# QZ1-boy/FCVSR

Measured on AMD Instinct MI355X. Metric: SR frames/sec (7-frame window, 4x 180x320->720x1280) + PSNR vs ref, higher is better.
Workload: dtype bf16

## Files before the change

fcvsr_amd/csrc/fft.hip:

```cpp
#include <stdlib.h>
#include <mutex>
#include "common.h"

namespace fcvsr {

struct FftPlan {
  int N;
  int nfac;
  int fac[20];
  unsigned magic[20];
};

static bool make_plan(int N, FftPlan* p) {
  p->N = N;
  p->nfac = 0;
  int n = N;
  while (n % 8 == 0) { p->fac[p->nfac++] = 8; n /= 8; }
  while (n % 4 == 0) { p->fac[p->nfac++] = 4; n /= 4; }
  while (n % 2 == 0) { p->fac[p->nfac++] = 2; n /= 2; }
  while (n % 9 == 0) { p->fac[p->nfac++] = 9; n /= 9; }
  for (int f = 3; f <= n; f += 2) {
    while (n % f == 0) {
      if (p->nfac >= 20) return false;
      p->fac[p->nfac++] = f;
// ... 153 lines not shown
  int cur = 0;
  int Ns = 1;
  for (int s = 0; s < plan.nfac; ++s) {
    const int r = plan.fac[s];
    const float* xr = lds + cur * 2 * NL;
    const float* xi = xr + NL;
    float* yr = lds + (cur ^ 1) * 2 * NL;
    float* yi = yr + NL;
    const unsigned mg = plan.magic[s];
    if (r == 8) stage_radix<8, INV>(xr, xi, yr, yi, tw, N, Ns, mg, L, logL);
    else if (r == 9) stage_radix<9, INV>(xr, xi, yr, yi, tw, N, Ns, mg, L, logL);
    else if (r == 4) stage_radix<4, INV>(xr, xi, yr, yi, tw, N, Ns, mg, L, logL);
    else if (r == 2) stage_radix<2, INV>(xr, xi, yr, yi, tw, N, Ns, mg, L, logL);
    else if (r == 3) stage_radix<3, INV>(xr, xi, yr, yi, tw, N, Ns, mg, L, logL);
    else if (r == 5) stage_radix<5, INV>(xr, xi, yr, yi, tw, N, Ns, mg, L, logL);
    else if (r > 1) stage_generic(xr, xi, yr, yi, tw, N, Ns, r, L, logL);
    if (r > 1) {
      __syncthreads();
      cur ^= 1;
    }
    Ns *= r;
  }
  return cur;
}

__device__ __forceinline__ void xcd_line_chunk(int* line, int* chunk) {
  const int nchunk = gridDim.x;
  const int lin = blockIdx.y * nchunk + blockIdx.x;
  const int grp = lin / (8 * nchunk), rem = lin - grp * (8 * nchunk);
  *line = grp * 8 + (rem & 7);
  *chunk = rem >> 3;
}

__device__ __forceinline__ float ld_act(const float* base, long long idx, int dt) {
  if (dt == FCVSR_F32) return base[idx];
  const unsigned short u = reinterpret_cast<const unsigned short*>(base)[idx];
  if (dt == FCVSR_BF16) return __uint_as_float((unsigned)u << 16);
  return (float)__builtin_bit_cast(_Float16, u);
}

__device__ __forceinline__ float4 ld_act4(const float* base, long long idx, int dt) {
  if (dt == FCVSR_F32) return *reinterpret_cast<const float4*>(base + idx);
  const uint2 v = *reinterpret_cast<const uint2*>(reinterpret_cast<const unsigned short*>(base) + idx);
  if (dt == FCVSR_BF16)
    return make_float4(__uint_as_float(v.x << 16), __uint_as_float(v.x & 0xffff0000u), __uint_as_float(v.y << 16),
                       __uint_as_float(v.y & 0xffff0000u));
  typedef __attribute__((ext_vector_type(2))) _Float16 h2;
  const h2 a = __builtin_bit_cast(h2, v.x), b = __builtin_bit_cast(h2, v.y);
  return make_float4((float)a[0], (float)a[1], (float)b[0], (float)b[1]);
}

__global__ __launch_bounds__(512) void rfft_rows_kernel(View src, int src_dt, int n, int H, int W, int L, float* spec,
                                                        long long ps, int im_off, int re_off, FftPlan plan, int vec, int nbatch) {
  extern __shared__ __align__(16) float lds[];
  const int NL = W * L;
  int row, chunk;
  xcd_line_chunk(&row, &chunk);
  const int b = row / H, y = row % H;
  if (b >= nbatch) return;
  const int c0 = chunk * 2 * L;
  const int Wf = W / 2 + 1;
  make_twiddles(lds + 4 * NL, W, false);
  const long long sp = (long long)b * src.sb + (long long)y * src.sy;
  const int logL = 31 - __clz(L);
  if (vec) {
    const int G4 = L >> 1;
// ... 372 lines not shown
      const float* mk = masks + (long long)m * N * Wf + kx;
      float mv[R1];
#pragma unroll
      for (int q = 0; q < R1; ++q) mv[q] = mk[(j + q * R2) * Wf];
      Cx v[R1];
#pragma unroll
      for (int q = 0; q < R1; ++q) v[q] = live ? Cx{raw[q].r * mv[q], raw[q].i * mv[q]} : Cx{0.f, 0.f};
      Dft<R1, true>::run(v);
#pragma unroll
      for (int p = 0; p < R1; ++p) {
        const int idx = (j * R1 + p) * L + l;
        zr[idx] = v[p].r;
        zi[idx] = v[p].i;
      }
    }
    __syncthreads();
    if (j < R1) {
      Cx v[R2];
      stage2_load<R1, R2, true>(zr, zi, tw, j, l, L, v);
      if (live) {
        float* ob = out + (long long)m * out_band_stride + col0;
#pragma unroll
        for (int p = 0; p < R2; ++p) {
          float* px = ob + (long long)(j + p * R1) * rstride;
          px[re_off] = v[p].r;
          px[im_off] = v[p].i;
        }
      }
    }
    __syncthreads();
  }
}

template <int DT>
__device__ __forceinline__ Cx ld_pair(const float* base, long long idx) {
  if (DT == FCVSR_F32) { const float2 v = *reinterpret_cast<const float2*>(base + idx); return Cx{v.x, v.y}; }
  const unsigned v = *reinterpret_cast<const unsigned*>(reinterpret_cast<const unsigned short*>(base) + idx);
  if (DT == FCVSR_BF16) return Cx{__uint_as_float(v << 16), __uint_as_float(v & 0xffff0000u)};
  typedef __attribute__((ext_vector_type(2))) _Float16 h2;
  const h2 h = __builtin_bit_cast(h2, v);
  return Cx{(float)h[0], (float)h[1]};
}

template <int R1, int R2, int SDT>
__global__ __launch_bounds__(512, 4) void rfft_rows2_kernel(View src, int n, int H, int logL, float* spec, long long ps,
                                                         int im_off, int re_off, const float2* twtab, int nbatch) {
  constexpr int N = R1 * R2, Wf = N / 2 + 1;
  extern __shared__ __align__(16) float lds[];
  const int L = 1 << logL;
  float* zr = lds;
  float* zi = lds + N * L;
  float2* tw = reinterpret_cast<float2*>(lds + 2 * N * L);
  int grp, chunk;
  xcd_line_chunk(&grp, &chunk);
  const int row0 = grp, nrows = nbatch * H;
  if (row0 >= nrows) return;
  load_twiddles(tw, twtab, N);
  const int l = threadIdx.x & (L - 1), j = threadIdx.x >> logL;
  const int ca = chunk * 2 * L + 2 * l;
  const bool live = ca < n && j < R2;
  const int lane_off = live ? j * (int)src.sx + 2 * l : 0;
  auto issue = [&](const int row, Cx* v) {
    const int b = row / H, y = row - b * H;
    const long long sp = (long long)b * src.sb + (long long)y * src.sy + chunk * 2 * L;
#pragma unroll
    for (int q = 0; q < R1; ++q) {
// ... 160 lines not shown
  return L;
}
static int ilog2(int v) { int r = 0; while ((1 << r) < v) ++r; return r; }

#define FCVSR_FFT2_DISPATCH(ts, CALL)                                                                        \
  do {                                                                                                       \
    switch ((ts).N) {                                                                                        \
      case 64: CALL(8, 8); break;     case 72: CALL(8, 9); break;     case 80: CALL(8, 10); break;           \
      case 96: CALL(8, 12); break;    case 128: CALL(8, 16); break;   case 144: CALL(12, 12); break;         \
      case 160: CALL(10, 16); break;  case 180: CALL(12, 15); break;  case 192: CALL(12, 16); break;         \
      case 240: CALL(15, 16); break;  case 256: CALL(16, 16); break;  case 320: CALL(16, 20); break;         \
    }                                                                                                        \
  } while (0)
#define FCVSR_FFT2_DISPATCH_COLS(ts, CALL)                                                                   \
  do {                                                                                                       \
    switch ((ts).N) {                                                                                        \
      case 64: CALL(8, 8); break;     case 72: CALL(8, 9); break;     case 80: CALL(8, 10); break;           \
      case 96: CALL(8, 12); break;    case 128: CALL(8, 16); break;   case 144: CALL(12, 12); break;         \
      case 160: CALL(10, 16); break;  case 180: CALL(12, 15); break;  case 192: CALL(12, 16); break;         \
      case 256: CALL(16, 16); break;                                                                         \
    }                                                                                                        \
  } while (0)
#define FCVSR_FFT2_DISPATCH_BANDS(ts, CALL)                                                                  \
  do {                                                                                                       \
    switch ((ts).N) {                                                                                        \
      case 64: CALL(8, 8); break;     case 72: CALL(8, 9); break;     case 80: CALL(8, 10); break;           \
      case 96: CALL(8, 12); break;    case 128: CALL(8, 16); break;   case 144: CALL(12, 12); break;         \
      case 160: CALL(10, 16); break;  case 180: CALL(12, 15); break;                                         \
    }                                                                                                        \
  } while (0)
static const TwoStage* two_stage_cols(int N) { return (N == 240 || N == 320) ? nullptr : two_stage(N); }
static const TwoStage* two_stage_bands(int N) { return (N == 192 || N == 240 || N == 256 || N == 320) ? nullptr : two_stage(N); }

static int launch_cols2(const TwoStage& ts, const float* in, float* out, long long ps, int im_off, int re_off, int n, int Wf,
                        int B, bool inverse, const float* mask, hipStream_t st) {
  const float2* tw = twiddle_table(ts.N, st);
  if (!tw) return FCVSR_E_ARG;
  const int L = pick_lanes2(ts, n), logL = ilog2(L);
  const int rmax = ts.R1 > ts.R2 ? ts.R1 : ts.R2;
  const dim3 grid(cdiv(n, L), (B * Wf + 7) / 8 * 8), block((rmax * L + 63) / 64 * 64);
  const size_t lds = 8ull * ts.N * L + 8ull * ts.N;
#define FCVSR_COLS2(A_, B_)                                                                                                 \
  if (inverse && mask) hipLaunchKernelGGL((fft_cols2_kernel<A_, B_, true, true>), grid, block, lds, st, in, out, ps, im_off, \
                                          re_off, n, Wf, logL, mask, tw, B);                                                 \
  else if (inverse) hipLaunchKernelGGL((fft_cols2_kernel<A_, B_, true, false>), grid, block, lds, st, in, out, ps, im_off,   \
                                       re_off, n, Wf, logL, mask, tw, B);                                                    \
  else hipLaunchKernelGGL((fft_cols2_kernel<A_, B_, false, false>), grid, block, lds, st, in, out, ps, im_off, re_off, n,   \
                          Wf, logL, mask, tw, B)
  FCVSR_FFT2_DISPATCH_COLS(ts, FCVSR_COLS2);
#undef FCVSR_COLS2
  return 0;
}

static int launch_cols2_bands(const TwoStage& ts, const float* in, float* out, long long out_band_stride, long long ps, int im_off,
                             int re_off, int n, int Wf, int B, const float* masks, int nm, hipStream_t st) {
  const float2* tw = twiddle_table(ts.N, st);
  if (!tw) return FCVSR_E_ARG;
  const int L = pick_lanes2(ts, n), logL = ilog2(L);
  const int rmax = ts.R1 > ts.R2 ? ts.R1 : ts.R2;
  const dim3 grid(cdiv(n, L), (B * Wf + 7) / 8 * 8), block((rmax * L + 63) / 64 * 64);
  const size_t lds = 8ull * ts.N * L + 8ull * ts.N;
#define FCVSR_COLS2B(A_, B_) \
  hipLaunchKernelGGL((fft_cols2_bands_kernel<A_, B_>), grid, block, lds, st, in, out, out_band_stride, ps, im_off, re_off, n, Wf, logL, masks, nm, tw, B)
  FCVSR_FFT2_DISPATCH_BANDS(ts, FCVSR_COLS2B);
#undef FCVSR_COLS2B
  return 0;
}

static int launch_rfft_rows2(const TwoStage& ts, const fcvsr_view* src, int n, int B, int H, float* spec, long long ps, int im_off,
                             int re_off, hipStream_t st) {
  const float2* tw = twiddle_table(ts.N, st);
  if (!tw) return FCVSR_E_ARG;
  const int L = pick_lanes2(ts, n / 2), logL = ilog2(L);
  const int rmax = ts.R1 > ts.R2 ? ts.R1 : ts.R2;
  const dim3 grid(cdiv(n, 2 * L), (B * H + 7) / 8 * 8), block((rmax * L + 63) / 64 * 64);
  const size_t lds = 8ull * ts.N * L + 8ull * ts.N;
#define FCVSR_ROWS2(A_, B_)                                                                                                      \
  if (src->dtype == FCVSR_F32)                                                                                                   \
    hipLaunchKernelGGL((rfft_rows2_kernel<A_, B_, FCVSR_F32>), grid, block, lds, st, to_view(*src), n, H, logL, spec, ps, im_off, \
                       re_off, tw, B);                                                                                           \
  else if (src->dtype == FCVSR_BF16)                                                                                             \
    hipLaunchKernelGGL((rfft_rows2_kernel<A_, B_, FCVSR_BF16>), grid, block, lds, st, to_view(*src), n, H, logL, spec, ps,       \
                       im_off, re_off, tw, B);                                                                                   \
  else                                                                                                                           \
    hipLaunchKernelGGL((rfft_rows2_kernel<A_, B_, FCVSR_F16>), grid, block, lds, st, to_view(*src), n, H, logL, spec, ps, im_off, \
                       re_off, tw, B)
  FCVSR_FFT2_DISPATCH(ts, FCVSR_ROWS2);
#undef FCVSR_ROWS2
  return 0;
}

static int launch_irfft_rows2(const TwoStage& ts, const float* spec, long long ps, int im_off, int re_off, int n, int B, int H,
                              const fcvsr_view* dst, float scale, hipStream_t st) {
  const float2* tw = twiddle_table(ts.N, st);
  if (!tw) return FCVSR_E_ARG;
  const int L = pick_lanes2(ts, n / 2), logL = ilog2(L);
  const int rmax = ts.R1 > ts.R2 ? ts.R1 : ts.R2;
  const dim3 grid(cdiv(n, 2 * L), (B * H + 7) / 8 * 8), block((rmax * L + 63) / 64 * 64);
  const size_t lds = 8ull * ts.N * L + 8ull * ts.N;
#define FCVSR_IROWS2(A_, B_) \
  hipLaunchKernelGGL((irfft_rows2_kernel<A_, B_>), grid, block, lds, st, spec, ps, im_off, re_off, n, H, logL, to_view(*dst), scale, tw, B)
  FCVSR_FFT2_DISPATCH(ts, FCVSR_IROWS2);
#undef FCVSR_IROWS2
  return 0;
}

static bool pair_ok(const fcvsr_view* v) {
  const int al = v->dtype == FCVSR_F32 ? 8 : 4;
  return v->sc == 1 && v->sx % 2 == 0 && v->sy % 2 == 0 && v->sb % 2 == 0 && ((uintptr_t)v->ptr % al) == 0;
}

constexpr long long kFftLdsBudget = 64 * 1024;

static int pick_lanes(int N, int n_lanes_needed) {
  int L = 32;
  while (L > 1 && (16ll * N * L + 8ll * N) > kFftLdsBudget) L >>= 1;
  while (L > 1 && L / 2 >= n_lanes_needed) L >>= 1;
  return L;
}

template <class K>
static hipError_t allow_lds(K kernel, size_t bytes) {
  return hipFuncSetAttribute((const void*)kernel, hipFuncAttributeMaxDynamicSharedMemorySize, (int)bytes);
}

}

using namespace fcvsr;

extern "C" int fcvsr_rfft2(const fcvsr_view* src, int B, int H, int W, int n, float* spec, int64_t pix_stride,
                           int im_off, int re_off, void* stream) {
  FCVSR_CHECK_ARG(src && src->ptr && spec, "null pointer");
  FCVSR_CHECK_ARG(src->dtype == FCVSR_F32 || src->dtype == FCVSR_BF16 || src->dtype == FCVSR_F16, "bad src dtype");
  FCVSR_CHECK_ARG(B > 0 && H > 0 && W > 1 && n > 0 && n <= src->c, "bad sizes");
  FftPlan pw, ph;
  FCVSR_CHECK_ARG(make_plan(W, &pw) && make_plan(H, &ph), "length has too many factors");
  const int Wf = W / 2 + 1;
  hipStream_t st = (hipStream_t)stream;
  const bool spec_ok = pix_stride % 4 == 0 && im_off % 4 == 0 && re_off % 4 == 0 && ((uintptr_t)spec % 16) == 0;
  const bool spec_pair = pix_stride % 2 == 0 && im_off % 2 == 0 && re_off % 2 == 0 && ((uintptr_t)spec % 8) == 0;
  const TwoStage* tsw = two_stage(W);
  const TwoStage* tsh = two_stage_cols(H);
  if (tsw && n % 2 == 0 && pair_ok(src) && spec_pair) {
    const int rc = launch_rfft_rows2(*tsw, src, n, B, H, spec, (long long)pix_stride, im_off, re_off, st);
    if (rc) return rc;
    FCVSR_LAUNCH_CHECK();
  } else {
    const int L = pick_lanes(W, (n + 1) / 2);
    FCVSR_CHECK_ARG(16ll * W * L + 8ll * W <= 160 * 1024, "row too long for LDS");
    const size_t lds = 16ull * W * L + 8ull * W;
    (void)allow_lds(rfft_rows_kernel, lds);
    dim3 grid(cdiv(n, 2 * L), (B * H + 7) / 8 * 8);
    const int sal = src->dtype == FCVSR_F32 ? 16 : 8;
    const int vec = (L >= 4 && n % (2 * L) == 0 && src->sc == 1 && src->sx % 4 == 0 && src->sy % 4 == 0 && src->sb % 4 == 0 &&
                     ((uintptr_t)src->ptr % sal) == 0 && spec_ok) ? 1 : 0;
    hipLaunchKernelGGL(rfft_rows_kernel, grid, dim3(512), lds, st, to_view(*src), (int)src->dtype, n, H, W, L, spec,
                       (long long)pix_stride, im_off, re_off, pw, vec, B);
    FCVSR_LAUNCH_CHECK();
  }
  if (tsh) {
    const int rc = launch_cols2(*tsh, spec, spec, (long long)pix_stride, im_off, re_off, n, Wf, B, false, nullptr, st);
    if (rc) return rc;
    FCVSR_LAUNCH_CHECK();
  } else {
    const int L = pick_lanes(H, n);
    FCVSR_CHECK_ARG(16ll * H * L + 8ll * H <= 160 * 1024, "column too long for LDS");
    const size_t lds = 16ull * H * L + 8ull * H;
    (void)allow_lds(fft_cols_kernel, lds);
    dim3 grid(cdiv(n, L), (B * Wf + 7) / 8 * 8);
    const int vec = (L >= 4 && n % L == 0 && spec_ok) ? 1 : 0;
    hipLaunchKernelGGL(fft_cols_kernel, grid, dim3(512), lds, st, (const float*)spec, spec, (long long)pix_stride, im_off,
                       re_off, n, H, Wf, L, 0, (const float*)nullptr, ph, vec, B);
    FCVSR_LAUNCH_CHECK();
  }
  return 0;
}

static int irfft_rows(const float* mid, long long pix_stride, int im_off, int re_off, int n, int B, int H, int W, const FftPlan& pw,
                      bool mid_vec, const fcvsr_view* dst, hipStream_t st) {
  const TwoStage* tsw = two_stage(W);
  const bool mid_pair = pix_stride % 2 == 0 && im_off % 2 == 0 && re_off % 2 == 0 && ((uintptr_t)mid % 8) == 0;
  if (tsw && n % 2 == 0 && pair_ok(dst) && mid_pair) {
    const int rc = launch_irfft_rows2(*tsw, mid, pix_stride, im_off, re_off, n, B, H, dst, 1.0f / ((float)H * (float)W), st);
    if (rc) return rc;
    FCVSR_LAUNCH_CHECK();
  } else {
    const int L = pick_lanes(W, (n + 1) / 2);
    FCVSR_CHECK_ARG(16ll * W * L + 8ll * W <= 160 * 1024, "row too long for LDS");
    const size_t lds = 16ull * W * L + 8ull * W;
    (void)allow_lds(irfft_rows_kernel, lds);
    dim3 grid(cdiv(n, 2 * L), (B * H + 7) / 8 * 8);
// ... 38 lines not shown

extern "C" int fcvsr_irfft2_bands(const float* spec, int64_t pix_stride, int im_off, int re_off, int B, int H, int W, int n,
                                  const float* masks, int n_bands, float* work, const fcvsr_view* dst, void* stream) {
  FCVSR_CHECK_ARG(spec && masks && work && dst && n_bands >= 1 && n_bands <= 16, "null argument / 1..16 bands");
  FCVSR_CHECK_ARG(B > 0 && H > 0 && W > 1 && n > 0, "bad sizes");
  const int Wf = W / 2 + 1;
  const long long band = (long long)B * H * Wf * pix_stride;
  hipStream_t st = (hipStream_t)stream;
  const TwoStage* tsh = two_stage_bands(H);
  if (!tsh) {
    for (int m = 0; m < n_bands; ++m) {
      const int rc = fcvsr_irfft2(spec, pix_stride, im_off, re_off, B, H, W, n, masks + (long long)m * H * Wf, work, &dst[m], stream);
      if (rc) return rc;
    }
    return 0;
  }
  for (int m = 0; m < n_bands; ++m)
    FCVSR_CHECK_ARG(dst[m].ptr && dst[m].dtype == FCVSR_F32 && n <= dst[m].c, "dst: f32 views with >= n channels");
  {
    const int rc = launch_cols2_bands(*tsh, spec, work, band, (long long)pix_stride, im_off, re_off, n, Wf, B, masks, n_bands, st);
    if (rc) return rc;
    FCVSR_LAUNCH_CHECK();
  }
  FftPlan pw;
  FCVSR_CHECK_ARG(make_plan(W, &pw), "length has too many factors");
  for (int m = 0; m < n_bands; ++m) {
    const float* mid = work + (long long)m * band;
    const bool mid_vec = pix_stride % 4 == 0 && im_off % 4 == 0 && re_off % 4 == 0 && ((uintptr_t)mid % 16) == 0;
    const int rc = irfft_rows(mid, (long long)pix_stride, im_off, re_off, n, B, H, W, pw, mid_vec, &dst[m], st);
    if (rc) return rc;
  }
  return 0;
}
```

fcvsr_amd/engine.py:

```python
from __future__ import annotations

import ctypes as C
import math
import weakref
from collections import OrderedDict
from typing import Dict, List, Optional, Tuple

import numpy as np
import torch

from . import hip
from .hip import ACT_LEAKY, ACT_NONE, ACT_PRELU, ACT_RELU, check, lib, ptr, stream_ptr, view


_MASKS: Dict[Tuple[int, int, int], torch.Tensor] = {}


def band_masks_half(Q: int, H: int, W: int) -> torch.Tensor:
    key = (Q, H, W)
    if key not in _MASKS:
        n = 1024
        step = math.sqrt((n / 2) ** 2 + (n / 2) ** 2) / Q
        d2 = (np.arange(-(n // 2), n - n // 2, 1) ** 2).astype(np.float64)
        r2 = np.power(np.sqrt(d2[:, None] + d2[None, :]), 2)
# ... 369 lines not shown
                    else:
                        s_v, v_v = view(s), view(vbuf)
                        check(L.fcvsr_warp(C.byref(cur_v), C.byref(o_v), B, H, W, C.byref(s_v), st), "fcvsr_warp")
                        check(L.fcvsr_sac_v(C.byref(s_v), C.byref(k_v), B, H, W, C.byref(v_v), st), "fcvsr_sac_v")
                        check(L.fcvsr_sac_h(C.byref(v_v), C.byref(k_v), C.byref(fv), 0.1, B, H, W, C.byref(d_v), st),
                              "fcvsr_sac_h")
                    cur = dst
        out = self._new(dev, B, H, W, n, dtype=fdt_act)
        self._conv("MGAA.conv3", [al], out, res=[x2])
        if self.taps is not None:
            self._tap(f"mgaa{tag}.off_f", off4[:B])
            self._tap(f"mgaa{tag}.off_b", off4[B:])
            self._tap(f"mgaa{tag}.sim", sim)
            o = offsets.permute(0, 3, 1, 2).reshape(B, 2, A, 2, H, W)
            self.taps[f"mgaa{tag}.offsets_f"] = o[:, 0].contiguous().clone()
            self.taps[f"mgaa{tag}.offsets_b"] = o[:, 1].contiguous().clone()
            self._tap(f"mgaa{tag}.al_f", al[..., :n])
            self._tap(f"mgaa{tag}.al_b", al[..., n:])
            self._tap(f"mgaa{tag}.out", out)
        return out

    def _mffr(self, x, out_dtype=torch.float32):
        m = self._model()
        n, Q = m.n_feats, m.Freq_Inv
        dev = x.device
        B, H, W, _ = x.shape
        Wf = W // 2 + 1
        L = lib()
        st = stream_ptr()
        par = self._par
        masks = self._mask(Q, H, W, dev)
        spec = self._new(dev, B, H, Wf, 2 * n)
        xv = view(x)
        check(L.fcvsr_rfft2(C.byref(xv), B, H, W, n, spec.data_ptr(), 2 * n, 0, n, st), "fcvsr_rfft2")
        bands = self._new(dev, Q, B, H, W, n)
        work = self._new(dev, Q, B, H, Wf, 2 * n)
        bvs = (hip.View * Q)(*[view(bands[q]) for q in range(Q)])
        check(L.fcvsr_irfft2_bands(spec.data_ptr(), 2 * n, 0, n, B, H, W, n, masks.data_ptr(), Q, work.data_ptr(), bvs, st),
              "fcvsr_irfft2_bands")
        freq = [bands[Q - 1 - i] for i in range(Q)]
        s_o = self._new(dev, B, H, W, n)
        nblk = (H * W + 255) // 256
        scratch = self._new(dev, 2 * B * nblk * n)
        sums = self._new(dev, 2, B, n)
        inv_hw = 1.0 / (H * W)
        mean_sum = self._channel_sum(freq[0])
        ab = [(par[f"MFFRblock.DivEnh_block.{i}.a"], par[f"MFFRblock.DivEnh_block.{i}.b"]) for i in range(Q)]
        staged = n % 4 == 0 and 256 % (n // 4) == 0 and all(f.data_ptr() % 16 == 0 for f in freq)
        s_f = self._new(dev, B, H, W, n) if (Q > 4 or not staged) else None
        check(L.fcvsr_divenh(0, 1, freq[0].data_ptr(), (s_f if s_f is not None else s_o).data_ptr(), s_o.data_ptr(),
                             ab[0][0].data_ptr(), ab[0][1].data_ptr(), mean_sum.data_ptr(), inv_hw, None, None, sums.data_ptr(),
                             scratch.data_ptr(), scratch.numel(), B, H, W, n, st), "fcvsr_divenh(reduce)")
        gates = []
        j0 = 0
        for i in range(Q):
            pre = f"MFFRblock.DivEnh_block.{i}"
            a, b = ab[i]
            first = 1 if i == 0 else 0
            g1 = self._ca_gate(sums[0], inv_hw, pre + ".ca", B, n)
            g2 = self._ca_gate(sums[1], inv_hw, pre + ".ca", B, n) if i > 0 else None
            gates.append((g1, g2))
            sums = self._new(dev, 2, B, n)
            nxt = i + 1 < Q
            if staged:
                sa = hip.DivEnhStageArgs()
                if j0 > 0:
                    sa.ck_s_f, sa.ck_s_o = s_f.data_ptr(), s_o.data_ptr()
                for k, j in enumerate(range(j0, i + 1)):
                    sa.f[k], sa.a[k], sa.b[k] = freq[j].data_ptr(), ab[j][0].data_ptr(), ab[j][1].data_ptr()
                    sa.g1[k], sa.g2[k] = gates[j][0].data_ptr(), ptr(gates[j][1])
                sa.mean_f_sum = mean_sum.data_ptr()
                if nxt:
# ... 381 lines not shown
```

fcvsr_amd/hip.py:

```python
from __future__ import annotations

import ctypes as C
import os
from typing import Optional, Sequence

import torch

_HERE = os.path.dirname(os.path.abspath(__file__))
LIB_PATH = os.path.join(_HERE, "lib", "libfcvsr_hip.so")

F32, BF16, F16, U8 = 0, 1, 2, 3
ACT_NONE, ACT_RELU, ACT_LEAKY, ACT_PRELU = 0, 1, 2, 3
_DT = {torch.float32: F32, torch.bfloat16: BF16, torch.float16: F16, torch.uint8: U8}


class View(C.Structure):
    _fields_ = [("ptr", C.c_void_p), ("sb", C.c_int64), ("sy", C.c_int64), ("sx", C.c_int64), ("sc", C.c_int64),
                ("c", C.c_int32), ("dtype", C.c_int32)]


class GcFinishLevel(C.Structure):
    _fields_ = [("partial", C.c_void_p), ("add", C.c_void_p), ("nparts", C.c_int32)]


# ... 2 lines not shown


class GcApplyLevel(C.Structure):
    _fields_ = [("r", C.c_void_p), ("add", C.c_void_p), ("z", C.c_void_p), ("out", C.c_void_p), ("pool", C.c_void_p),
                ("B", C.c_int32), ("H", C.c_int32), ("W", C.c_int32)]


class XscaleLevel(C.Structure):
    _fields_ = [("x", C.c_void_p), ("r", C.c_void_p), ("dn", C.c_void_p), ("up", C.c_void_p), ("out", C.c_void_p),
                ("r_scale", C.c_float), ("dn_pooled", C.c_int32), ("B", C.c_int32), ("H", C.c_int32), ("W", C.c_int32)]


class RcbTailArgs(C.Structure):
    _fields_ = [("x", C.c_void_p * 3), ("r", C.c_void_p * 3), ("z", C.c_void_p * 3), ("add", C.c_void_p * 3),
                ("out", C.c_void_p * 3), ("r1", C.c_void_p), ("u1", C.c_void_p), ("u2", C.c_void_p), ("w_up", C.c_void_p),
                ("b_up", C.c_void_p), ("w_dn", C.c_void_p), ("b_dn", C.c_void_p), ("B", C.c_int32), ("H", C.c_int32),
                ("W", C.c_int32)]


class DivEnhStageArgs(C.Structure):
    _fields_ = [("ck_s_f", C.c_void_p), ("ck_s_o", C.c_void_p), ("f", C.c_void_p * 4), ("a", C.c_void_p * 4),
                ("b", C.c_void_p * 4), ("g1", C.c_void_p * 4), ("g2", C.c_void_p * 4), ("mean_f_sum", C.c_void_p),
                ("f_next", C.c_void_p), ("a_next", C.c_void_p), ("b_next", C.c_void_p), ("out_s_f", C.c_void_p),
                ("out_s_o", C.c_void_p), ("sums", C.c_void_p), ("scratch", C.c_void_p), ("scratch_elems", C.c_int64),
                ("inv_hw", C.c_float), ("n_bands", C.c_int32), ("B", C.c_int32), ("H", C.c_int32), ("W", C.c_int32),
                ("C", C.c_int32)]


class CropDesc(C.Structure):
    _fields_ = [("src", C.c_void_p), ("pitch", C.c_int32), ("top", C.c_int32), ("left", C.c_int32), ("flags", C.c_int32)]


CROP_HFLIP, CROP_VFLIP, CROP_TRANSPOSE = 1, 2, 4


class ConvDesc(C.Structure):
    _fields_ = [("n_src", C.c_int32), ("src", View * 3), ("B", C.c_int32), ("H", C.c_int32), ("W", C.c_int32),
                ("kh", C.c_int32), ("kw", C.c_int32), ("stride", C.c_int32), ("pad", C.c_int32),
                ("cout", C.c_int32), ("weight", C.c_void_p), ("cout_pad", C.c_int32), ("bias", C.c_void_p),
                ("act", C.c_int32), ("slope", C.c_float), ("slope_ptr", C.c_void_p), ("n_res", C.c_int32),
                ("res", View * 2), ("res_scale", C.c_float * 2), ("dst", View), ("pixel_shuffle", C.c_int32),
                ("gc_wmask", C.c_void_p), ("gc_partial", C.c_void_p)]


PROFILE = None
COMPUTE_DTYPE = "f32"
DOMINANT_KERNEL = "conv_direct_kernel"


class HipError(RuntimeError):
    pass


_lib: Optional[C.CDLL] = None

_VP, _I, _I64, _F = C.c_void_p, C.c_int, C.c_int64, C.c_float
_PV = C.POINTER(View)
SIGNATURES = {
    "fcvsr_last_error": [],
    "fcvsr_last_conv_kernel": [],
    "fcvsr_conv2d_wgrad_scratch_elems": [C.c_int] * 7,
    "fcvsr_conv2d_wgrad": [C.c_void_p, C.c_void_p, C.c_int, C.c_int, C.c_int, C.c_int, C.c_int, C.c_int, C.c_int, C.c_void_p, C.c_void_p,
                           C.c_longlong, C.c_int, C.c_void_p],
    "fcvsr_conv2d_wgrad_mfma_eligible": [C.c_int] * 6,
    "fcvsr_conv2d_wgrad_mfma_scratch_elems": [C.c_int] * 7,
    "fcvsr_conv2d_wgrad_mfma": [C.c_void_p, C.c_void_p, C.c_int, C.c_int, C.c_int, C.c_int, C.c_int, C.c_int, C.c_int, C.c_void_p, C.c_void_p,
                                C.c_void_p, C.c_longlong, C.c_int, C.c_int, C.c_void_p],
    "fcvsr_abi_version": [],
    "fcvsr_device_count": [],
    "fcvsr_conv2d": [C.POINTER(ConvDesc), _VP],
    "fcvsr_conv2d_f32mfma": [C.POINTER(ConvDesc), _VP],
    "fcvsr_conv2d_f32mfma_eligible": [C.POINTER(ConvDesc)],
    "fcvsr_conv2d_mfma": [C.POINTER(ConvDesc), _I, _I, _VP],
    "fcvsr_conv2d_mfma_plan": [C.POINTER(ConvDesc), _I, _I, _I, _I, C.c_char_p, _I],
    "fcvsr_rfft2": [_PV, _I, _I, _I, _I, _VP, _I64, _I, _I, _VP],
    "fcvsr_irfft2": [_VP, _I64, _I, _I, _I, _I, _I, _I, _VP, _VP, _PV, _VP],
    "fcvsr_irfft2_bands": [_VP, _I64, _I, _I, _I, _I, _I, _I, _VP, _I, _VP, _PV, _VP],
    "fcvsr_corr_lookup": [_VP, _VP, _I64, _I, _I, _I, _I, _I, _I, _PV, _VP],
    "fcvsr_channel_sum": [_PV, _I, _I, _I, _VP, _VP, _I64, _VP],
    "fcvsr_ca_gate": [_VP, _F, _VP, _VP, _I, _I, _I, _VP, _VP],
    "fcvsr_convblk_tail": [_VP, _VP, _VP, _I, _I, _I, _I, _VP, _I64, _I, _I, _I, _I, _VP],
    "fcvsr_convblk": [_VP, _VP, _VP, _VP, _I, _VP, _VP, _VP, _I, _I, _I, _I, _VP, _VP, _I64, _VP, _I64, _I, _I, _I, _I, _VP],
    "fcvsr_warp": [_PV, _PV, _I, _I, _I, _PV, _VP],
    "fcvsr_sac_v": [_PV, _PV, _I, _I, _I, _PV, _VP],
    "fcvsr_sac_h": [_PV, _PV, _PV, _F, _I, _I, _I, _PV, _VP],
    "fcvsr_iac_step": [_PV, _PV, _PV, _PV, _F, _I, _I, _I, _PV, _VP],
    "fcvsr_feat_extract": [_PV, _I, _I, _I, _VP, _VP, _I, _VP, _VP, _VP, _I, _VP],
    "fcvsr_freq_head": [_VP, _I, _I64, _I64, _VP, _VP, _VP, _VP, _VP],
    "fcvsr_freq_mlp3": [_VP, _VP, _I, _I64, _I64, _VP, _VP, _VP, _VP, _I64, _VP],
    "fcvsr_iac_step2": [_PV, _PV, _PV, _PV, _F, _I, _I, _I, _PV, _VP],
    "fcvsr_iac_step2_fused": [_PV, _PV, _PV, _VP, _VP, _PV, _F, _I, _I, _I, _PV, _VP],
    "fcvsr_divenh": [_I, _I, _VP, _VP, _VP, _VP, _VP, _VP, _F, _VP, _VP, _VP, _VP, _I64, _I, _I, _I, _I, _VP],
    "fcvsr_divenh_apply_next": [_I, _VP, _VP, _VP, _VP, _VP, _VP, _F, _VP, _VP, _VP, _VP, _VP, _VP, _VP, _I64, _I, _I, _I, _I, _VP],
    "fcvsr_divenh_stage": [C.POINTER(DivEnhStageArgs), _VP],
    "fcvsr_scale_add": [_VP, _VP, _VP, _I, _VP, _I, _I, _I, _I, _I, _VP],
    "fcvsr_gc_context": [_VP, _VP, _VP, _VP, _I, _I, _I, _I, _VP, _VP, _I64, _VP],
    "fcvsr_gc_finish": [_VP, _I, _VP, _VP, _I, _I, _VP, _VP],
    "fcvsr_gc_apply": [_VP, _VP, _VP, _VP, _I, _F, _I, _I, _I, _I, _VP],
    "fcvsr_xscale": [_VP, _VP, _F, _VP, _VP, _VP, _I, _I, _I, _I, _I, _VP],
    "fcvsr_gc_finish_levels": [C.POINTER(GcFinishLevel), _I, _VP, _VP, _I, _I, _VP],
    "fcvsr_gc_partial_levels": [C.POINTER(GcPartialLevel), _I, _I, _VP, _I, _VP],
    "fcvsr_gc_apply_levels": [C.POINTER(GcApplyLevel), _I, _I, _I, _F, _I, _VP],
    "fcvsr_xscale_levels": [C.POINTER(XscaleLevel), _I, _I, _I, _VP],
    "fcvsr_rcb_level0": [_VP, _VP, _VP, _VP, _VP, _VP, _VP, _F, _F, _I, _I, _I, _I, _I, _VP],
    "fcvsr_rcb_tail": [C.POINTER(RcbTailArgs), _F, _I, _I, _VP],
    "fcvsr_pixel_shuffle": [_VP, _VP, _I, _I, _I, _I, _VP],
    "fcvsr_pixel_shuffle16": [_VP, _PV, _I, _I, _I, _I, _VP],
    "fcvsr_bilinear_up4": [_PV, _I, _I, _I, _PV, _VP],
    "fcvsr_tail_fused": [_PV, _VP, _VP, _VP, _VP, _VP, _I, _I, _I, _PV, _VP],
    "fcvsr_tail_fused_base": [_PV, _VP, _VP, _VP, _VP, _VP, _PV, _I, _I, _I, _PV, _VP],
# ... 303 lines not shown
```

include/fcvsr_hip.h:

```cpp
#ifndef FCVSR_HIP_H
#define FCVSR_HIP_H

#include <stddef.h>
#include <stdint.h>

#ifdef __cplusplus
extern "C" {
#endif

#define FCVSR_ABI_VERSION 2

enum { FCVSR_E_ARG = -1, FCVSR_E_UNSUPPORTED = -2, FCVSR_E_NOGPU = -3 };
enum { FCVSR_F32 = 0, FCVSR_BF16 = 1, FCVSR_F16 = 2 };
enum { FCVSR_U8 = 3 };
enum { FCVSR_ACT_NONE = 0, FCVSR_ACT_RELU = 1, FCVSR_ACT_LEAKY = 2, FCVSR_ACT_PRELU = 3 };

typedef struct fcvsr_view {
  void*   ptr;
  int64_t sb, sy, sx, sc;
  int32_t c;
  int32_t dtype;
} fcvsr_view;

typedef struct fcvsr_conv_desc {
// ... 57 lines not shown
                              const float* w2, int B, int HW, int C, float* sf_out, float* so_out, float* stats, float* scratch,
                              long long scratch_elems, void* stream);
int fcvsr_divenh_band_backward(const float* f, const float* sf, const float* so, const float* a, const float* b, const float* w1,
                               const float* w2, const float* stats, const float* gsf, const float* gso, int B, int HW, int C, float* gf,
                               float* gsf_out, float* gso_out, float* ga, float* gb, float* dw1, float* dw2, float* scratch,
                               long long scratch_elems, int accumulate, void* stream);
int fcvsr_corr_lookup_bwd(const float* x1f, const float* x2f, int64_t pix_stride, int B, int H, int Wf, int C, int radius, int x_count,
                          const fcvsr_view* g, float* gx1_zeroed, float* gx2_zeroed, void* stream);
int fcvsr_prelu_fwd(const float* x, const float* slope, float* y, long long n, void* stream);
int fcvsr_prelu_bwd(const float* g, const float* x, const float* slope, float* gx, float* gslope, float* scratch, long long n, void* stream);
long long fcvsr_wgrad_cout1_scratch_elems(int B, int H, int C);
int fcvsr_wgrad_cout1(const float* x, const float* gy, int B, int H, int W, int C, float* dw, float* scratch, long long scratch_elems,
                      int accumulate, void* stream);
int fcvsr_iac_bwd_sac(const float* gy, const float* yout, const float* v, const float* s, const fcvsr_view* k1, float slope, int B, int H,
                      int W, int C, float* gfin, int fin_accumulate, float* gv, const fcvsr_view* gk, int k_accumulate, void* stream);
int fcvsr_iac_bwd_warp(const float* gv, const fcvsr_view* k1, const float* prev, const fcvsr_view* off, int B, int H, int W, int C,
                       float* gprev_zeroed, float* goff, void* stream);
int fcvsr_iac_bwd_warp_det_workspace(int B, int H, int W, int C, size_t* bytes);
int fcvsr_iac_bwd_warp_det(const float* gv, const fcvsr_view* k1, const float* prev, const fcvsr_view* off, int B, int H, int W, int C,
                           float* gprev, float* goff, void* workspace, size_t workspace_bytes, void* stream);
long long fcvsr_conv2d_wgrad_mfma_groups_scratch_elems(const int* B, const int* H, const int* W, int n_groups, int cin, int cout, int kh,
                                                       int kw);
int fcvsr_conv2d_wgrad_mfma_groups(const fcvsr_view* xs, const fcvsr_view* gys, const int* B, const int* H, const int* W, int n_groups, int kh,
                                   int kw, int pad, float* dw, float* dbias, float* scratch, long long scratch_elems, int dw_accumulate,
                                   int dbias_accumulate, void* stream);
int fcvsr_up2_adjoint(const float* g, float* out, int B, int H, int W, int C, void* stream);
int fcvsr_pool2_adjoint(const float* g, float* out, int B, int H, int W, int C, void* stream);
int fcvsr_rfft2(const fcvsr_view* src, int B, int H, int W, int n,
                float* spec, int64_t pix_stride, int im_off, int re_off, void* stream);
int fcvsr_irfft2(const float* spec, int64_t pix_stride, int im_off, int re_off, int B, int H, int W, int n,
                 const float* mask, float* work, const fcvsr_view* dst, void* stream);
int fcvsr_irfft2_bands(const float* spec, int64_t pix_stride, int im_off, int re_off, int B, int H, int W, int n,
                       const float* masks, int n_bands, float* work, const fcvsr_view* dst, void* stream);

int fcvsr_feat_extract(const fcvsr_view* x, int B, int H, int W, const void* w, const float* bias, int n_blk,
                       void* const* dst, const int64_t* dst_pix_stride, const int32_t* dst_ch_off, int dst_dtype,
                       void* stream);

int fcvsr_corr_lookup(const float* x1f, const float* x2f, int64_t pix_stride, int B, int H, int Wf, int C, int radius,
                      int x_count, const fcvsr_view* dst, void* stream);
int fcvsr_channel_sum(const fcvsr_view* src, int B, int H, int W, float* out, float* scratch, int64_t scratch_elems,
                      void* stream);
int fcvsr_ca_gate(const float* sum, float inv_hw, const float* w1, const float* w2, int B, int c, int cr,
                  float* gate, void* stream);
int fcvsr_convblk_tail(const float* u, const float* gate, const float* sim, int B, int ndir, int H, int Wf,
                       float* spec, int64_t pix_stride, int re_off, int im_off, int g_stride, int g0, void* stream);
int fcvsr_convblk(const float* x, const float* w1, const float* w2, const float* prelu_slope, int ksize, const float* ca_w1,
                  const float* ca_w2, const float* sim, int B, int ndir, int H, int Wf, float* u_scratch,
                  float* partial_scratch, int64_t partial_elems, float* spec, int64_t pix_stride, int re_off, int im_off,
                  int g_stride, int g0, void* stream);
int fcvsr_warp(const fcvsr_view* src, const fcvsr_view* off, int B, int H, int W, const fcvsr_view* dst, void* stream);
int fcvsr_sac_v(const fcvsr_view* s, const fcvsr_view* k1, int B, int H, int W, const fcvsr_view* dst, void* stream);
int fcvsr_sac_h(const fcvsr_view* v, const fcvsr_view* k1, const fcvsr_view* feat_in, float slope,
                int B, int H, int W, const fcvsr_view* dst, void* stream);

int fcvsr_iac_step(const fcvsr_view* prev, const fcvsr_view* off, const fcvsr_view* k1, const fcvsr_view* feat_in,
                   float slope, int B, int H, int W, const fcvsr_view* dst, void* stream);
int fcvsr_iac_step2(const fcvsr_view* prev, const fcvsr_view* off, const fcvsr_view* k1, const fcvsr_view* feat_in,
                    float slope, int B, int H, int W, const fcvsr_view* dst, void* stream);
int fcvsr_iac_step2_fused(const fcvsr_view* prev, const fcvsr_view* off, const fcvsr_view* k0, const void* wk,
                          const float* kbias, const fcvsr_view* feat_in, float slope, int B, int H, int W,
                          const fcvsr_view* dst, void* stream);

int fcvsr_freq_mlp3(const float* const* xa, const float* const* xb, int n_dirs, int64_t src_pix_stride, int64_t npix,
                    const void* w0, const void* w2, const void* w4, void* const* dst, int64_t dst_pix_stride, void* stream);

// ... 143 lines not shown
```

Measured before the change: 899.1.

## Fuse forward column FFT with per-band masked inverse column FFT in persistent kernel

Adds a fused kernel that performs the forward column FFT and then, for each frequency band, applies the mask and the inverse column FFT while the spectrum stays in LDS/registers. This removes one full spectrum write and read per call. The kernel uses a persistent grid sized to the CU count, assigns line ranges per XCD, and prefetches the next column and mask loads to overlap memory with compute. It adds extra synchronisation per band and fixes occupancy at four waves per SIMD, which may limit parallelism when there are few lines.

After: 901.0 (median of 6 runs). Within noise of the previous version (+0.2%).

```diff
diff --git a/fcvsr_amd/csrc/fft.hip b/fcvsr_amd/csrc/fft.hip
--- a/fcvsr_amd/csrc/fft.hip
+++ b/fcvsr_amd/csrc/fft.hip
@@ -209,6 +209,30 @@
   *chunk = rem >> 3;
 }
 
+__device__ __forceinline__ int fresh_tid() {
+  int t = threadIdx.x;
+  asm volatile("" : "+v"(t));
+  return t;
+}
+__device__ __forceinline__ void fft_arrived(float v) { asm volatile("" ::"v"(v)); }
+__device__ __forceinline__ void fft_arrived(Cx v) { asm volatile("" ::"v"(v.r), "v"(v.i)); }
+#define FCVSR_FFT_LANE() const int tid_ = fresh_tid(); const int l = tid_ & (L - 1), j = tid_ >> logL; (void)l; (void)j
+struct FftRun { int line0, unit0, count; };
+__host__ __device__ __forceinline__ FftRun fft_wg_run(int lines, int nchunk, int nwg, int wg) {
+  FftRun r = {0, 0, 0};
+  const int nx = lines < 8 ? lines : 8;
+  const int S = nwg < 8 ? 1 : nwg >> 3;
+  const int xcd = wg & 7, slot = wg >> 3;
+  if (xcd >= nx || slot >= S || wg >= nwg) return r;
+  const int base = lines / nx, rem = lines - base * nx;
+  const int lx = base + (xcd < rem ? 1 : 0);
+  r.line0 = xcd * base + (xcd < rem ? xcd : rem);
+  const int U = lx * nchunk, ub = U / S, ur = U - ub * S;
+  r.count = ub + (slot < ur ? 1 : 0);
+  r.unit0 = slot * ub + (slot < ur ? slot : ur);
+  return r;
+}
+
 __device__ __forceinline__ float ld_act(const float* base, long long idx, int dt) {
   if (dt == FCVSR_F32) return base[idx];
   const unsigned short u = reinterpret_cast<const unsigned short*>(base)[idx];
@@ -647,6 +671,155 @@
   }
 }
 
+template <int R1, int R2>
+__global__ __launch_bounds__(512) __attribute__((amdgpu_waves_per_eu(4, 4)))
+void fft_cols2_fwd_bands_kernel(const float* in, float* out, long long out_band_stride, long long ps, int im_off, int re_off, int n,
+                                int Wf, int logL, const float* masks, int nm, const float2* twtab, int nlines, int nchunk) {
+  constexpr int N = R1 * R2;
+  extern __shared__ __align__(16) float lds[];
+  const int L = 1 << logL;
+  float* zr = lds;
+  float* zi = lds + N * L;
+  float2* tw = reinterpret_cast<float2*>(lds + 2 * N * L);
+  const FftRun run = fft_wg_run(nlines, nchunk, gridDim.x, blockIdx.x);
+  if (run.count <= 0) return;
+  load_twiddles(tw, twtab, N);
+  const long long rstride = (long long)Wf * ps;
+  Cx nxt[R1];
+  float mv[R1];
+  auto locate = [&](int col, int chunk, int* kx) {
+    const int b = col / Wf;
+    *kx = col - b * Wf;
+    return ((long long)b * N * Wf + *kx) * ps + chunk * L;
+  };
+  auto issue_in = [&](long long col0, int chunk) {
+    FCVSR_FFT_LANE();
+    if (j < R2) {
+      const int lo = chunk * L + l < n ? l : 0;
+#pragma unroll
+      for (int q = 0; q < R1; ++q) {
+        const float* px = in + col0 + (long long)(j + q * R2) * rstride + lo;
+        nxt[q] = Cx{px[re_off], px[im_off]};
+      }
+    }
+  };
+  auto issue_mask = [&](int m, int kx) {
+    FCVSR_FFT_LANE();
+    if (j < R2) {
+      const float* mk = masks + (long long)m * N * Wf + kx;
+#pragma unroll
+      for (int q = 0; q < R1; ++q) mv[q] = mk[(j + q * R2) * Wf];
+    }
+  };
+  const int ul = run.unit0 / nchunk;
+  int col = run.line0 + ul, chunk = run.unit0 - ul * nchunk, kx;
+  long long col0 = locate(col, chunk, &kx);
+  issue_in(col0, chunk);
+  issue_mask(0, kx);
+  for (int it = 0; it < run.count; ++it) {
+    const bool more = it + 1 < run.count;
+    {
+      FCVSR_FFT_LANE();
+      if (j < R2) {
+        const bool live = chunk * L + l < n;
+        Cx v[R1];
+#pragma unroll
+        for (int q = 0; q < R1; ++q) v[q] = live ? nxt[q] : Cx{0.f, 0.f};
+        Dft<R1, false>::run(v);
+#pragma unroll
+        for (int p = 0; p < R1; ++p) {
+          const int idx = (j * R1 + p) * L + l;
+          zr[idx] = v[p].r;
+          zi[idx] = v[p].i;
+        }
+      }
+    }
+#pragma unroll
+    for (int q = 0; q < R1; ++q) fft_arrived(nxt[q]);
+    __syncthreads();
+    {
+      FCVSR_FFT_LANE();
+      if (j < R1) {
+        Cx w[R2];
+        stage2_load<R1, R2, false>(zr, zi, tw, j, l, L, w);
+#pragma unroll
+        for (int p = 0; p < R2; ++p) {
+          const int idx = (j + p * R1) * L + l;
+          zr[idx] = w[p].r;
+          zi[idx] = w[p].i;
+        }
+      }
+    }
+    __syncthreads();
+    Cx raw[R1];
+    {
+      FCVSR_FFT_LANE();
+      if (j < R2) {
+#pragma unroll
+        for (int q = 0; q < R1; ++q) {
+          const int idx = (j + q * R2) * L + l;
+          raw[q] = Cx{zr[idx], zi[idx]};
+        }
+      }
+    }
+    __syncthreads();
+    long long ncol0 = col0;
+    int ncol = col, nchk = chunk, nkx = kx;
+    auto band = [&](const int m, const bool last) {
+      {
+        FCVSR_FFT_LANE();
+        if (j < R2) {
+          const bool live = chunk * L + l < n;
+          Cx v[R1];
+#pragma unroll
+          for (int q = 0; q < R1; ++q) v[q] = live ? Cx{raw[q].r * mv[q], raw[q].i * mv[q]} : Cx{0.f, 0.f};
+          Dft<R1, true>::run(v);
+#pragma unroll
+          for (int p = 0; p < R1; ++p) {
+            const int idx = (j * R1 + p) * L + l;
+            zr[idx] = v[p].r;
+            zi[idx] = v[p].i;
+          }
+        }
+      }
+#pragma unroll
+      for (int q = 0; q < R1; ++q) fft_arrived(mv[q]);
+      __syncthreads();
+      if (last && more) {
+        if (++nchk == nchunk) { nchk = 0; ++ncol; }
+        ncol0 = locate(ncol, nchk, &nkx);
+        issue_in(ncol0, nchk);
+      }
+      Cx v[R2];
+      {
+        FCVSR_FFT_LANE();
+        if (j < R1) stage2_load<R1, R2, true>(zr, zi, tw, j, l, L, v);
+      }
+      if (!last) issue_mask(m + 1, kx);
+      else if (more) issue_mask(0, nkx);
+      {
+        FCVSR_FFT_LANE();
+        if (j < R1 && chunk * L + l < n) {
+          float* ob = out + (long long)m * out_band_stride + col0 + l;
+#pragma unroll
+          for (int p = 0; p < R2; ++p) {
+            float* px = ob + (long long)(j + p * R1) * rstride;
+            px[re_off] = v[p].r;
+            px[im_off] = v[p].i;
+          }
+        }
+      }
+      if (!last || more) __syncthreads();
+    };
+    for (int m = 0; m + 1 < nm; ++m) band(m, false);
+    band(nm - 1, true);
+    kx = nkx;
+    col0 = ncol0;
+    col = ncol;
+    chunk = nchk;
+  }
+}
+
 template <int DT>
 __device__ __forceinline__ Cx ld_pair(const float* base, long long idx) {
   if (DT == FCVSR_F32) { const float2 v = *reinterpret_cast<const float2*>(base + idx); return Cx{v.x, v.y}; }
@@ -873,6 +1046,46 @@
 static const TwoStage* two_stage_cols(int N) { return (N == 240 || N == 320) ? nullptr : two_stage(N); }
 static const TwoStage* two_stage_bands(int N) { return (N == 192 || N == 240 || N == 256 || N == 320) ? nullptr : two_stage(N); }
 
+static const int kFftWavesPerSimd[FCVSR_FFT_KINDS] = {4};
+
+static const TwoStage* two_stage_kind(int kind, int N) {
+  switch (kind) {
+    case FCVSR_FFT_COLS_FWD_BANDS: return two_stage_bands(N);
+  }
+  return nullptr;
+}
+
+static bool fft_plan(int kind, int N, int lanes_needed, int lines, int cus, fcvsr_fft_plan_t* p) {
+  const TwoStage* ts = two_stage_kind(kind, N);
+  if (!ts || lanes_needed < 1 || lines < 1) return false;
+  const int rmax = ts->R1 > ts->R2 ? ts->R1 : ts->R2;
+  p->lanes = pick_lanes2(*ts, lanes_needed);
+  p->chunks = cdiv(lanes_needed, p->lanes);
+  p->threads = (rmax * p->lanes + 63) / 64 * 64;
+  p->lds_bytes = 8 * ts->N * p->lanes + 8 * ts->N;
+  int per_cu = 160 * 1024 / p->lds_bytes;
+  const int by_waves = kFftWavesPerSimd[kind] * 4 / (p->threads / 64);
+  if (by_waves < per_cu) per_cu = by_waves;
+  p->per_cu = per_cu < 1 ? 1 : (per_cu > 8 ? 8 : per_cu);
+  if (cus < 1) cus = 256;
+  if (lines < 8) {
+    p->workgroups = lines;
+  } else {
+    int slots = p->per_cu * cus / 8;
+    const int most = (lines / 8) * p->chunks;
+    if (slots > most) slots = most;
+    if (slots < 1) slots = 1;
+    p->workgroups = 8 * slots;
+  }
+  return true;
+}
+
+static bool fft_plan_here(int kind, int N, int lanes_needed, int lines, fcvsr_fft_plan_t* p) {
+  int dev = 0;
+  if (hipGetDevice(&dev) != hipSuccess) dev = -1;
+  return fft_plan(kind, N, lanes_needed, lines, dev >= 0 ? device_cu_count(dev) : 0, p);
+}
+
 static int launch_cols2(const TwoStage& ts, const float* in, float* out, long long ps, int im_off, int re_off, int n, int Wf,
                         int B, bool inverse, const float* mask, hipStream_t st) {
   const float2* tw = twiddle_table(ts.N, st);
@@ -905,6 +1118,23 @@
   hipLaunchKernelGGL((fft_cols2_bands_kernel<A_, B_>), grid, block, lds, st, in, out, out_band_stride, ps, im_off, re_off, n, Wf, logL, masks, nm, tw, B)
   FCVSR_FFT2_DISPATCH_BANDS(ts, FCVSR_COLS2B);
 #undef FCVSR_COLS2B
+  return 0;
+}
+
+static int launch_cols2_fwd_bands(const TwoStage& ts, const float* in, float* out, long long out_band_stride, long long ps,
+                                  int im_off, int re_off, int n, int Wf, int B, const float* masks, int nm, hipStream_t st) {
+  const float2* tw = twiddle_table(ts.N, st);
+  if (!tw) return FCVSR_E_ARG;
+  fcvsr_fft_plan_t pl;
+  if (!fft_plan_here(FCVSR_FFT_COLS_FWD_BANDS, ts.N, n, B * Wf, &pl)) return FCVSR_E_ARG;
+  const int logL = ilog2(pl.lanes), nl = B * Wf;
+  const dim3 grid(pl.workgroups), block(pl.threads);
+  const size_t lds = pl.lds_bytes;
+#define FCVSR_COLS2FB(A_, B_)                                                                                                  \
+  hipLaunchKernelGGL((fft_cols2_fwd_bands_kernel<A_, B_>), grid, block, lds, st, in, out, out_band_stride, ps, im_off, re_off, \
+                     n, Wf, logL, masks, nm, tw, nl, pl.chunks)
+  FCVSR_FFT2_DISPATCH_BANDS(ts, FCVSR_COLS2FB);
+#undef FCVSR_COLS2FB
   return 0;
 }
 
@@ -969,21 +1199,12 @@
 
 using namespace fcvsr;
 
-extern "C" int fcvsr_rfft2(const fcvsr_view* src, int B, int H, int W, int n, float* spec, int64_t pix_stride,
-                           int im_off, int re_off, void* stream) {
-  FCVSR_CHECK_ARG(src && src->ptr && spec, "null pointer");
-  FCVSR_CHECK_ARG(src->dtype == FCVSR_F32 || src->dtype == FCVSR_BF16 || src->dtype == FCVSR_F16, "bad src dtype");
-  FCVSR_CHECK_ARG(B > 0 && H > 0 && W > 1 && n > 0 && n <= src->c, "bad sizes");
-  FftPlan pw, ph;
-  FCVSR_CHECK_ARG(make_plan(W, &pw) && make_plan(H, &ph), "length has too many factors");
-  const int Wf = W / 2 + 1;
-  hipStream_t st = (hipStream_t)stream;
-  const bool spec_ok = pix_stride % 4 == 0 && im_off % 4 == 0 && re_off % 4 == 0 && ((uintptr_t)spec % 16) == 0;
+static int rfft_rows(const fcvsr_view* src, int B, int H, int W, int n, float* spec, long long pix_stride, int im_off, int re_off,
+                     const FftPlan& pw, bool spec_ok, hipStream_t st) {
   const bool spec_pair = pix_stride % 2 == 0 && im_off % 2 == 0 && re_off % 2 == 0 && ((uintptr_t)spec % 8) == 0;
   const TwoStage* tsw = two_stage(W);
-  const TwoStage* tsh = two_stage_cols(H);
   if (tsw && n % 2 == 0 && pair_ok(src) && spec_pair) {
-    const int rc = launch_rfft_rows2(*tsw, src, n, B, H, spec, (long long)pix_stride, im_off, re_off, st);
+    const int rc = launch_rfft_rows2(*tsw, src, n, B, H, spec, pix_stride, im_off, re_off, st);
     if (rc) return rc;
     FCVSR_LAUNCH_CHECK();
   } else {
@@ -996,8 +1217,42 @@
     const int vec = (L >= 4 && n % (2 * L) == 0 && src->sc == 1 && src->sx % 4 == 0 && src->sy % 4 == 0 && src->sb % 4 == 0 &&
                      ((uintptr_t)src->ptr % sal) == 0 && spec_ok) ? 1 : 0;
     hipLaunchKernelGGL(rfft_rows_kernel, grid, dim3(512), lds, st, to_view(*src), (int)src->dtype, n, H, W, L, spec,
-                       (long long)pix_stride, im_off, re_off, pw, vec, B);
+                       pix_stride, im_off, re_off, pw, vec, B);
     FCVSR_LAUNCH_CHECK();
+  }
+  return 0;
+}
+
+extern "C" int fcvsr_fft_plan(int kind, int N, int lanes_needed, int lines, int cus, fcvsr_fft_plan_t* plan) {
+  FCVSR_CHECK_ARG(plan && kind >= 0 && kind < FCVSR_FFT_KINDS, "null plan / unknown kind");
+  FCVSR_CHECK_ARG(fft_plan(kind, N, lanes_needed, lines, cus, plan), "no two-stage kernel of this kind for the length, or bad sizes");
+  return 0;
+}
+
+extern "C" int fcvsr_fft_plan_unit(const fcvsr_fft_plan_t* plan, int lines, int wg, int iter, int* line, int* chunk) {
+  FCVSR_CHECK_ARG(plan && line && chunk && lines > 0 && wg >= 0 && iter >= 0 && plan->chunks > 0, "bad argument");
+  const FftRun r = fft_wg_run(lines, plan->chunks, plan->workgroups, wg);
+  if (iter >= r.count) return 1;
+  const int u = r.unit0 + iter;
+  *line = r.line0 + u / plan->chunks;
+  *chunk = u % plan->chunks;
+  return 0;
+}
+
+extern "C" int fcvsr_rfft2(const fcvsr_view* src, int B, int H, int W, int n, float* spec, int64_t pix_stride,
+                           int im_off, int re_off, void* stream) {
+  FCVSR_CHECK_ARG(src && src->ptr && spec, "null pointer");
+  FCVSR_CHECK_ARG(src->dtype == FCVSR_F32 || src->dtype == FCVSR_BF16 || src->dtype == FCVSR_F16, "bad src dtype");
+  FCVSR_CHECK_ARG(B > 0 && H > 0 && W > 1 && n > 0 && n <= src->c, "bad sizes");
+  FftPlan pw, ph;
+  FCVSR_CHECK_ARG(make_plan(W, &pw) && make_plan(H, &ph), "length has too many factors");
+  const int Wf = W / 2 + 1;
+  hipStream_t st = (hipStream_t)stream;
+  const bool spec_ok = pix_stride % 4 == 0 && im_off % 4 == 0 && re_off % 4 == 0 && ((uintptr_t)spec % 16) == 0;
+  const TwoStage* tsh = two_stage_cols(H);
+  {
+    const int rc = rfft_rows(src, B, H, W, n, spec, (long long)pix_stride, im_off, re_off, pw, spec_ok, st);
+    if (rc) return rc;
   }
   if (tsh) {
     const int rc = launch_cols2(*tsh, spec, spec, (long long)pix_stride, im_off, re_off, n, Wf, B, false, nullptr, st);
@@ -1102,3 +1357,36 @@
   }
   return 0;
 }
+
+extern "C" int fcvsr_rfft2_bands(const fcvsr_view* src, int B, int H, int W, int n, float* scratch, const float* masks, int n_bands,
+                                 float* work, const fcvsr_view* dst, void* stream) {
+  FCVSR_CHECK_ARG(src && src->ptr && scratch && masks && work && dst && n_bands >= 1 && n_bands <= 16, "null argument / 1..16 bands");
+  FCVSR_CHECK_ARG(src->dtype == FCVSR_F32 || src->dtype == FCVSR_BF16 || src->dtype == FCVSR_F16, "bad src dtype");
+  FCVSR_CHECK_ARG(B > 0 && H > 0 && W > 1 && n > 0 && n <= src->c, "bad sizes");
+  const TwoStage* tsh = two_stage_bands(H);
+  FCVSR_CHECK_ARG(tsh, "no fused column pass for this height (use fcvsr_rfft2 + fcvsr_irfft2_bands)");
+  for (int m = 0; m < n_bands; ++m)
+    FCVSR_CHECK_ARG(dst[m].ptr && dst[m].dtype == FCVSR_F32 && n <= dst[m].c, "dst: f32 views with >= n channels");
+  FftPlan pw;
+  FCVSR_CHECK_ARG(make_plan(W, &pw), "length has too many factors");
+  const int Wf = W / 2 + 1, im_off = 0, re_off = n;
+  const long long ps = 2ll * n, band = (long long)B * H * Wf * ps;
+  hipStream_t st = (hipStream_t)stream;
+  {
+    const bool ok = ps % 4 == 0 && re_off % 4 == 0 && ((uintptr_t)scratch % 16) == 0;
+    const int rc = rfft_rows(src, B, H, W, n, scratch, ps, im_off, re_off, pw, ok, st);
+    if (rc) return rc;
+  }
+  {
+    const int rc = launch_cols2_fwd_bands(*tsh, scratch, work, band, ps, im_off, re_off, n, Wf, B, masks, n_bands, st);
+    if (rc) return rc;
+    FCVSR_LAUNCH_CHECK();
+  }
+  for (int m = 0; m < n_bands; ++m) {
+    const float* mid = work + (long long)m * band;
+    const bool mid_vec = ps % 4 == 0 && re_off % 4 == 0 && ((uintptr_t)mid % 16) == 0;
+    const int rc = irfft_rows(mid, ps, im_off, re_off, n, B, H, W, pw, mid_vec, &dst[m], st);
+    if (rc) return rc;
+  }
+  return 0;
+}
diff --git a/fcvsr_amd/engine.py b/fcvsr_amd/engine.py
--- a/fcvsr_amd/engine.py
+++ b/fcvsr_amd/engine.py
@@ -425,12 +425,16 @@
         masks = self._mask(Q, H, W, dev)
         spec = self._new(dev, B, H, Wf, 2 * n)
         xv = view(x)
-        check(L.fcvsr_rfft2(C.byref(xv), B, H, W, n, spec.data_ptr(), 2 * n, 0, n, st), "fcvsr_rfft2")
         bands = self._new(dev, Q, B, H, W, n)
         work = self._new(dev, Q, B, H, Wf, 2 * n)
         bvs = (hip.View * Q)(*[view(bands[q]) for q in range(Q)])
-        check(L.fcvsr_irfft2_bands(spec.data_ptr(), 2 * n, 0, n, B, H, W, n, masks.data_ptr(), Q, work.data_ptr(), bvs, st),
-              "fcvsr_irfft2_bands")
+        if H in hip.FFT_BANDS_HEIGHTS:
+            check(L.fcvsr_rfft2_bands(C.byref(xv), B, H, W, n, spec.data_ptr(), masks.data_ptr(), Q, work.data_ptr(), bvs, st),
+                  "fcvsr_rfft2_bands")
+        else:
+            check(L.fcvsr_rfft2(C.byref(xv), B, H, W, n, spec.data_ptr(), 2 * n, 0, n, st), "fcvsr_rfft2")
+            check(L.fcvsr_irfft2_bands(spec.data_ptr(), 2 * n, 0, n, B, H, W, n, masks.data_ptr(), Q, work.data_ptr(), bvs, st),
+                  "fcvsr_irfft2_bands")
         freq = [bands[Q - 1 - i] for i in range(Q)]
         s_o = self._new(dev, B, H, W, n)
         nblk = (H * W + 255) // 256
diff --git a/fcvsr_amd/hip.py b/fcvsr_amd/hip.py
--- a/fcvsr_amd/hip.py
+++ b/fcvsr_amd/hip.py
@@ -58,6 +58,15 @@
 
 
 CROP_HFLIP, CROP_VFLIP, CROP_TRANSPOSE = 1, 2, 4
+
+
+class FftPlan(C.Structure):
+    _fields_ = [("lanes", C.c_int32), ("chunks", C.c_int32), ("workgroups", C.c_int32), ("lds_bytes", C.c_int32),
+                ("threads", C.c_int32), ("per_cu", C.c_int32)]
+
+
+FFT_COLS_FWD_BANDS = 0
+FFT_BANDS_HEIGHTS = (64, 72, 80, 96, 128, 144, 160, 180)
 
 
 class ConvDesc(C.Structure):
@@ -102,6 +111,9 @@
     "fcvsr_rfft2": [_PV, _I, _I, _I, _I, _VP, _I64, _I, _I, _VP],
     "fcvsr_irfft2": [_VP, _I64, _I, _I, _I, _I, _I, _I, _VP, _VP, _PV, _VP],
     "fcvsr_irfft2_bands": [_VP, _I64, _I, _I, _I, _I, _I, _I, _VP, _I, _VP, _PV, _VP],
+    "fcvsr_rfft2_bands": [_PV, _I, _I, _I, _I, _VP, _VP, _I, _VP, _PV, _VP],
+    "fcvsr_fft_plan": [_I, _I, _I, _I, _I, _VP],
+    "fcvsr_fft_plan_unit": [_VP, _I, _I, _I, C.POINTER(C.c_int), C.POINTER(C.c_int)],
     "fcvsr_corr_lookup": [_VP, _VP, _I64, _I, _I, _I, _I, _I, _I, _PV, _VP],
     "fcvsr_channel_sum": [_PV, _I, _I, _I, _VP, _VP, _I64, _VP],
     "fcvsr_ca_gate": [_VP, _F, _VP, _VP, _I, _I, _I, _VP, _VP],
diff --git a/include/fcvsr_hip.h b/include/fcvsr_hip.h
--- a/include/fcvsr_hip.h
+++ b/include/fcvsr_hip.h
@@ -113,6 +113,13 @@
                  const float* mask, float* work, const fcvsr_view* dst, void* stream);
 int fcvsr_irfft2_bands(const float* spec, int64_t pix_stride, int im_off, int re_off, int B, int H, int W, int n,
                        const float* masks, int n_bands, float* work, const fcvsr_view* dst, void* stream);
+int fcvsr_rfft2_bands(const fcvsr_view* src, int B, int H, int W, int n, float* scratch, const float* masks, int n_bands,
+                      float* work, const fcvsr_view* dst, void* stream);
+#define FCVSR_FFT_COLS_FWD_BANDS 0
+#define FCVSR_FFT_KINDS 1
+typedef struct fcvsr_fft_plan_t { int lanes, chunks, workgroups, lds_bytes, threads, per_cu; } fcvsr_fft_plan_t;
+int fcvsr_fft_plan(int kind, int N, int lanes_needed, int lines, int cus, fcvsr_fft_plan_t* plan);
+int fcvsr_fft_plan_unit(const fcvsr_fft_plan_t* plan, int lines, int wg, int iter, int* line, int* chunk);
 
 int fcvsr_feat_extract(const fcvsr_view* x, int B, int H, int W, const void* w, const float* bias, int n_blk,
                        void* const* dst, const int64_t* dst_pix_stride, const int32_t* dst_ch_off, int dst_dtype,
```
